# leggedrobotics/elevation_mapping_cupy

Measured on AMD Instinct MI355X. Metric: Mpoints/s fused (map-update p50 latency in config), higher is better.
Workload: dtype f32; 1 GPU; cfg2: 1024x1024 map, 1000000 uniform-random points/frame, core_param.yaml values, add_points + variance fusion, rays/overlap off; index_mode=reference_fp16, cloud=device resident (H2D excluded)

## Files before the change

elevation_mapping_cupy_amd/csrc/emap_api.hip:

```cpp
#include "emap_host.h"
#include <algorithm>
#include <cmath>
#include <cstdio>
#include <cstdlib>
#include <cstring>
#include <new>

using namespace emap_host;

float emap_host::q16(float x) { return (float)(_Float16)x; }
static int frame_impl(emap_ctx* ctx, const float R[9], const float t[3], double position_noise, double orientation_noise, emap_stats* stats, bool sharded);
static void sf_forget_applied(emap_ctx* ctx) {
  const unsigned int passed = ctx->sf_host[0];
  while (ctx->sf_count > 0 && ctx->sf_ring[ctx->sf_head].epoch <= passed) { ctx->sf_head = (ctx->sf_head + 1) % emap_ctx::SF_RING; --ctx->sf_count; }
}
static int sf_recover(emap_ctx* ctx) {
  CK(hipSetDevice(ctx->device));
  CK(hipStreamSynchronize(ctx->stream));
  const unsigned int first = ctx->sf_host[1];
  ctx->sf_host[1] = 0u;
  CK(hipMemset(ctx->sf_poison, 0, 4));
  const BoundCloud bound = ctx->cloud;
  const bool fsem_set = ctx->fsem_set; ctx->fsem_set = false;
  int rc = EMAP_OK;
// ... 242 lines not shown
  hipFree(s->dev);
  *s = Stage{};
}

extern "C" {

int emap_abi_version(void) { return EMAP_ABI_VERSION; }

const char* emap_last_error(const emap_ctx* ctx) { return ctx ? ctx->err.c_str() : "null context"; }

int emap_destroy(emap_ctx* ctx) {
  if (!ctx) return EMAP_OK;
  hipSetDevice(ctx->device);
  if (ctx->post_pending) post_settle(ctx);
  if (ctx->stream) hipStreamSynchronize(ctx->stream);
  hipFree(ctx->cells.hot); hipFree(ctx->cells.cold); hipFree(ctx->acc); hipFree(ctx->accr); hipFree(ctx->trav_in);
  hipFree(ctx->normal); hipFree(ctx->scratch); hipFree(ctx->plug_buf); hipFree(ctx->plug_cnt); hipFree(ctx->slots); hipFree(ctx->frame); hipFree(ctx->cnt_sync);
  for (int k = 0; k < 2; ++k) { hipFree(ctx->pts_dev[k]); if (ctx->pts_pin[k]) hipHostFree(ctx->pts_pin[k]); if (ctx->ev_copied[k]) hipEventDestroy(ctx->ev_copied[k]); if (ctx->ev_used[k]) hipEventDestroy(ctx->ev_used[k]); }
  hipFree(ctx->own_cloud); stage_free(&ctx->cloud_stage); stage_free(&ctx->image_stage);
  if (ctx->copy_stream) hipStreamDestroy(ctx->copy_stream);
  delete ctx->workers;
  hipFree(ctx->tail_idx); hipFree(ctx->tail_flags); hipFree(ctx->ray_S); hipFree(ctx->ray_lut); hipFree(ctx->inert); hipFree(ctx->inl_plane); hipFree(ctx->ray_thr);
  hipFree(ctx->bin_recs); hipFree(ctx->bin_own); hipFree(ctx->bin_own_cnt); hipFree(ctx->bin_hist); hipFree(ctx->bin_tile_total); hipFree(ctx->bin_tile_start); hipFree(ctx->bin_sync); hipFree(ctx->split_mem); hipFree(ctx->sem_split_mem); if (ctx->split_need) hipHostFree((void*)ctx->split_need); if (ctx->sf_host) hipHostFree((void*)ctx->sf_host); hipFree(ctx->frame_save); hipFree(ctx->sf_poison);
  hipFree(ctx->img_uv); hipFree(ctx->img_valid); hipFree(ctx->img_buf);
  hipFree(ctx->grid_buf);
  hipFree(ctx->poly_buf); if (ctx->poly_pin) hipHostFree(ctx->poly_pin);
  hipFree(ctx->sub_tab); hipFree(ctx->sub_out); if (ctx->sub_pin) hipHostFree(ctx->sub_pin);
  hipFree(ctx->cloud_tab); hipFree(ctx->cloud_out); if (ctx->cloud_pin) hipHostFree(ctx->cloud_pin);
  hipFree(ctx->pseg_buf); hipFree(ctx->pseg_slots); if (ctx->pseg_pin) hipHostFree(ctx->pseg_pin);
  hipFree(ctx->terr_buf); if (ctx->terr_pin) hipHostFree(ctx->terr_pin);
  hipFree(ctx->reg_buf); hipFree(ctx->reg_cracks); if (ctx->reg_pin) hipHostFree(ctx->reg_pin);
// ... 397 lines not shown
  if (ctx->pts_bucketed) {
    CKARG(memcmp(ctx->bucket_R, R, sizeof ctx->bucket_R) == 0 && memcmp(ctx->bucket_t, t, sizeof ctx->bucket_t) == 0, "the bound cloud was bucketed for another pose (emap_upload_points_strip)");
    CKARG(ctx->bucket_org_r == ctx->kp.org_r, "the map's rows shifted since the bound cloud was bucketed for this strip (emap_upload_points_strip): upload it again");
  }
  const bool gate_possible = !f || f->gate_possible;
  ctx->bin_rs = 1;
  CK(hipSetDevice(ctx->device));
  const bool binned = ctx->cloud.n > 0 && takes_bins(ctx, ctx->cloud.n_all);
  ctx->frame_binned = binned;
  const bool tm = ctx->stage_timing && f;
  if (binned) {
    int rc = ensure_bins(ctx, ctx->prm.enable_visibility_cleanup != 0, f); if (rc) return rc;
    const Pose pose = make_pose(ctx, R, t);
    BinStg* own = ctx->bin_strip ? reinterpret_cast<BinStg*>(ctx->bin_own) : nullptr;
    if (tm) CK(hipEventRecord(ctx->ev[ST_HIST], ctx->stream));
    bool hist_done = false;
    if (ctx->post_pending) {
      const bool along = f && !tm && !own && ctx->kp.mv.n == 0;
      const bool rays_on = ctx->prm.enable_visibility_cleanup != 0;
      int out = POST_OUT_FULL;
      if (along) {
        out = rays_on ? POST_OUT_TRAV_NORMALS : POST_OUT_TRAV;
        if (const char* e = getenv("EMAP_POST_LEAN")) { if (atoi(e) == 0) out = POST_OUT_FULL; }
      }
      if (along && out == POST_OUT_TRAV && !gate_possible) ctx->post_took = 32;
      else {
        if (along) {
          long max_wg = 0;
          if (const char* e = getenv("EMAP_POST_FUSE_MAX_WG")) max_wg = atol(e);
          hist_done = launch_post_hist(ctx->stream, ctx->device, ctx->kp, ctx->prm.w1, ctx->prm.w2, ctx->prm.w3, ctx->prm.w_out, ctx->cells, ctx->trav_in, ctx->normal,
                                       ctx->ncells_alloc, ctx->prm.dilation_size, pose, ctx->bg, ctx->cloud.pts, ctx->cloud.n, ctx->cloud.stride, ctx->bin_hist, max_wg, out);
        }
        if (hist_done) {
          ++ctx->post_fused;
          if (out == POST_OUT_FULL) ctx->post_pending = false; else ctx->post_took = 16;
          if (out != POST_OUT_TRAV) { ctx->kp.norg_r = ctx->kp.org_r; ctx->kp.norg_c = ctx->kp.org_c; }
          if (out == POST_OUT_FULL) { ctx->torg_r = ctx->kp.org_r; ctx->torg_c = ctx->kp.org_c; }
        } else if ((rc = post_settle(ctx))) return rc;
      }
    }
    if (!hist_done) launch_bin_hist(ctx->stream, ctx->kp, pose, ctx->bg, ctx->cloud.pts, ctx->cloud.n, ctx->cloud.stride, ctx->bin_hist, own, ctx->bin_own_cnt);
    if (tm) CK(hipEventRecord(ctx->ev[ST_SCAN], ctx->stream));
    static const bool split_off = getenv("EMAP_SPLIT") && atoi(getenv("EMAP_SPLIT")) == 0;
    ctx->split.on = gate_possible && !split_off ? 1 : 0;
    {
      static const int cap_forced = getenv("EMAP_SPLIT_CAP") ? atoi(getenv("EMAP_SPLIT_CAP")) : -1;
      static const int pool = getenv("EMAP_SPLIT_POOL") ? atoi(getenv("EMAP_SPLIT_POOL")) : EMAP_SPLIT_POOL_DEFAULT;
      const unsigned int need = *ctx->split_need;
      long cap = need ? (long)need + need / 4 + 8 : 0;
      if (ctx->split.on && cap < pool) cap = pool;
      if (cap_forced >= 0) cap = cap_forced;
      if (cap > (long)SPLIT_MAX_EXTRA) cap = SPLIT_MAX_EXTRA;
      ctx->split.cap = (int)((cap + 7) & ~7L);
    }
    if (ctx->split.on && ctx->split_dirty) {
      CK(hipMemsetAsync(ctx->split_mem, 0, (size_t)SPLIT_MAX_SLOTS * SPLIT_CELLS * 40 + 4 * SPLIT_MAX_SLOTS, ctx->stream));
      ctx->split_dirty = false;
    }
    ctx->split_dirty = ctx->split_dirty || (ctx->split.on != 0 && ctx->split.cap > 0);
    launch_bin_scan(ctx->stream, ctx->bg, ctx->bin_hist, ctx->bin_tile_total, ctx->bin_tile_start, ctx->bin_sync, ctx->split);
    if (tm) CK(hipEventRecord(ctx->ev[ST_SCATTER], ctx->stream));
    launch_bin_scatter(ctx->stream, ctx->kp, pose, ctx->bg, ctx->cloud.pts, ctx->cloud.n, ctx->cloud.stride, ctx->bin_hist, ctx->bin_tile_start, ctx->bin_recs, own, ctx->bin_own_cnt,
                       ctx->cloud.chan, ctx->carry);
    if (tm) CK(hipEventRecord(ctx->ev[ST_GATE], ctx->stream));
    if (gate_possible) launch_tile_count(ctx->stream, ctx->kp, ctx->bg, ctx->bin_recs, ctx->bin_rs, ctx->bin_tile_start, ctx->cells, ctx->slots, ctx->split, ctx->cloud.n);
  } else {
    { const int rc = post_settle(ctx); if (rc) return rc; }
    ctx->carry.on = 0;
    if (tm) for (int e = ST_HIST; e <= ST_SCATTER; ++e) CK(hipEventRecord(ctx->ev[e], ctx->stream));
    static const bool fold_off = getenv("EMAP_GATE_FOLD") && atoi(getenv("EMAP_GATE_FOLD")) == 0;
    const bool fold = f && f->fold_gate && !fold_off && ctx->cnt_sync;
    const bool folded = launch_count(ctx->stream, ctx->kp, make_pose(ctx, R, t), ctx->cloud.pts, ctx->cloud.n, ctx->cloud.stride, ctx->cells, ctx->acc, ctx->slots,
                                     fold ? &f->gate : nullptr, ctx->frame, ctx->cnt_sync);
    if (gate_folded) *gate_folded = folded;
    if (tm) CK(hipEventRecord(ctx->ev[ST_GATE], ctx->stream));
  }
  CK(hipGetLastError());
  return EMAP_OK;
}

// ... 440 lines not shown
```

elevation_mapping_cupy_amd/csrc/emap_binned.hip:

```cpp
#include "emap_launch.h"
#include "emap_bin_hist.h"
#include <cstring>
#include <cstdlib>

#define BIN_QCAP 128


template <int MODE> __device__ __forceinline__ bool row_owned(const KP& P, const Pose& T, float rx, float ry, float rz) {
  const float qx = Qf<MODE>(rx), qy = Qf<MODE>(ry), qz = Qf<MODE>(rz);
  const float x = T.Rq[0] * qx + T.Rq[1] * qy + T.Rq[2] * qz + T.tq[0];
  const int ix = axis_idx<MODE>(P, Qf<MODE>(x));
  return (unsigned int)(phys_row(P, ix) - P.row0) < (unsigned int)P.nrows;
}

struct __attribute__((aligned(16))) BinStg { unsigned int key; float z, v; unsigned int i; };

template <int MODE, int BLK, bool STRIP>
__global__ __launch_bounds__(BLK) void k_bin_hist(KP P, Pose T, BinGeo G, const float* __restrict__ pts, long n, int stride,
                                                  unsigned int* __restrict__ hist, BinStg* __restrict__ stg,
                                                  unsigned int* __restrict__ stg_cnt) {
  extern __shared__ __attribute__((aligned(16))) unsigned int h[];
  if (!STRIP) bin_hist_chunk<MODE, BLK, HIST_U>(P, T, G, pts, n, stride, hist, h, blockIdx.x, gridDim.x);
  else {
    for (int t = threadIdx.x; t < G.TB; t += BLK) h[t] = 0u;
// ... 227 lines not shown
  const unsigned int R0 = tile_start[w.t], R1 = tile_start[w.t + 1], n = R1 - R0;
  w.np = 1u; w.slot = SPLIT_NONE; w.r0 = R0; w.r1 = R1;
  if (SPLIT && n > SPLIT_CAP) {
    const unsigned int sw = SV.tile_slot[w.t];
    if (sw != SPLIT_NONE) {
      w.np = sw >> 16; w.slot = (sw & 0xffffu) + (unsigned int)w.sb;
      const unsigned int len = (n + w.np - 1u) / w.np;
      w.r0 = min(R1, R0 + w.part * len); w.r1 = min(R1, w.r0 + len);
    }
  }
  return true;
}

__device__ __forceinline__ bool drift_inlier(const KP& P, const float4 m, float z) {
  return m.z > 0.5f && (double)fabsf(m.x - z) < (double)m.y * P.mt && (double)m.y < P.dcvi_half && (double)m.w > P.trav_inlier;
}

#define TF_BLOCK 1024
#ifndef SPLIT_U
#define SPLIT_U 4
#endif
#ifndef SPLIT_U_FUSE
#define SPLIT_U_FUSE 1
#endif
__device__ __forceinline__ void stage_hot_tile(const KP& P, Cells cells, float4* s_cell, int row_base, int tx) {
  const int tr = __builtin_amdgcn_readfirstlane(threadIdx.x >> 6), tc = threadIdx.x & 63, lrow = row_base + tr, col = tx * BIN_TC + tc;
  const bool in = lrow < P.nrows && col < P.C;
  const float4* src = cells.hot + ((long)(lrow + P.halo) * P.C + col);
  if (P.mv.n == 0) {
    if (in) lds_dma16(src, s_cell + tr * BIN_TC);
    else s_cell[threadIdx.x] = make_float4(0.f, 0.f, 0.f, 0.f);
  } else {
    float4 m = make_float4(0.f, 0.f, 0.f, 0.f);
    if (in) { m = *src; cell_now(P, m, P.row0 + lrow, col); }
    s_cell[threadIdx.x] = m;
  }
}
template <bool SPLIT, int RS>
__device__ __forceinline__ void tile_count_body(const KP& P, const BinGeo& G, const BinRec* __restrict__ recs, Cells cells,
                                                ErrSlot* __restrict__ slots, const SplitView& SV, const TileWork& w) {
  constexpr int NC = BIN_TR * BIN_TC;
  __shared__ float4 s_cell[NC];
  __shared__ unsigned int s_pts[NC], s_inl[NC];
  const int t = w.t, sb = w.sb;
  const int ty = t / G.tiles_x, tx = t - ty * G.tiles_x;
  const unsigned int r0 = w.r0, r1 = w.r1;
  const int row_base = (ty * G.sub + sb) * BIN_TR;
  if (row_base >= P.nrows || r0 == r1) return;
  const bool split = SPLIT && w.np > 1u;
  constexpr int U = SPLIT ? SPLIT_U : 1;
  BinRec rr[U];
#pragma unroll
  for (int u = 0; u < U; ++u) { const unsigned int k = r0 + u * TF_BLOCK + threadIdx.x; if (k < r1) rr[u] = recs[(size_t)k * RS]; }
  stage_hot_tile(P, cells, s_cell, row_base, tx);
  if (split) { s_pts[threadIdx.x] = 0u; s_inl[threadIdx.x] = 0u; }
  __syncthreads();
  const unsigned int sel = (unsigned int)sb;
  for (unsigned int kb = r0; kb < r1; kb += TF_BLOCK * U) {
    if (kb != r0)
#pragma unroll
    for (int u = 0; u < U; ++u) { const unsigned int k = kb + u * TF_BLOCK + threadIdx.x; if (k < r1) rr[u] = recs[(size_t)k * RS]; }
    long long e_fix = 0; unsigned long long cnt = 0;
#pragma unroll
    for (int u = 0; u < U; ++u) {
      const unsigned int k = kb + u * TF_BLOCK + threadIdx.x;
      bool inl = false;
      if (k < r1) {
        const BinRec& r = rr[u];
        const unsigned int lcb = r.lc_inl & 0x7fffffffu;
        if ((lcb >> 10) == sel) {
          const float4 m = s_cell[lcb & 1023u];
          if (drift_inlier(P, m, r.z)) { inl = true; e_fix += __double2ll_rn((double)(r.z - m.x) * EM_SCALE_E); }
          if (split) { atomicAdd(&s_pts[lcb & 1023u], 1u); if (inl) atomicAdd(&s_inl[lcb & 1023u], 1u); }
        }
      }
      cnt += __popcll(__ballot(inl));
    }
    if (cnt) {
      const long long s = wave_sum_ll(e_fix);
      if ((threadIdx.x & 63) == 0) {
        const unsigned int slot = (unsigned int)(((unsigned int)t * (TF_BLOCK / 64) + (threadIdx.x >> 6) + kb) & (EM_ERR_SLOTS - 1));
        atomicAdd(reinterpret_cast<unsigned long long*>(&slots[slot].sum), (unsigned long long)s);
        atomicAdd(&slots[slot].cnt, cnt);
      }
    }
  }
  if (split) {
    __syncthreads();
    const unsigned int i = w.slot * SPLIT_CELLS + threadIdx.x;
    if (s_pts[threadIdx.x]) atomicAdd(&SV.pts[i], s_pts[threadIdx.x]);
    if (s_inl[threadIdx.x]) atomicAdd(&SV.inl[i], s_inl[threadIdx.x]);
  }
}
template <bool SPLIT, int RS>
__global__ __launch_bounds__(TF_BLOCK) void k_tile_count(KP P, BinGeo G, const BinRec* __restrict__ recs,
                                                          const unsigned int* __restrict__ tile_start, Cells cells,
                                                          ErrSlot* __restrict__ slots, SplitView SV) {
  TileWork w;
  if (tile_work<SPLIT>(G, SV, tile_start, w)) tile_count_body<SPLIT, RS>(P, G, recs, cells, slots, SV, w);
}

template <bool AVG, bool RAYS, bool SPLIT, int RS, bool SEM>
__device__ __forceinline__ void tile_fuse_body(const KP& P, const BinGeo& G, const BinRec* __restrict__ recs, Cells cells,
                                               AccF* __restrict__ acc, FrameDev* __restrict__ F,
                                               unsigned int* __restrict__ cnt_plane, unsigned long long* __restrict__ inert,
                                               unsigned int* __restrict__ inl_plane, float* __restrict__ thr, const OverlapArgs& O, const GateFold& GF,
                                               const SplitView& SV, const TileWork& w, const SemMini& SM) {
  static_assert(!SEM || (AVG && !RAYS && !SPLIT && RS == 2), "the semantic pass rides on whole frames without rays / parts, on 32-byte records");
  constexpr int NC = BIN_TR * BIN_TC;
  struct FuseLds { unsigned int pts[NC], cnt[NC], inl[NC], out[NC]; unsigned long long h[NC], v[NC], latest[NC]; float4 cell[NC]; };
  static_assert(offsetof(FuseLds, cell) == offsetof(FuseLds, h) + 3 * NC * 8 && sizeof(FuseLds) == 56 * NC, "FuseLds is packed");
  __shared__ __attribute__((aligned(16))) FuseLds L;
  unsigned int (&s_pts)[NC] = L.pts; unsigned int (&s_inl)[NC] = L.inl; unsigned int (&s_cnt)[NC] = L.cnt; unsigned int (&s_out)[NC] = L.out;
  unsigned long long (&s_h)[NC] = L.h; unsigned long long (&s_v)[NC] = L.v; unsigned long long (&s_latest)[NC] = L.latest;
// ... 286 lines not shown
  if (own) { if (P.mode == 0) launch_bin_scatter_i<0, BLK, true, false>(s, P, T, G, pts, n, stride, hist, tile_start, recs, own, own_cnt, V, SC); else launch_bin_scatter_i<1, BLK, true, false>(s, P, T, G, pts, n, stride, hist, tile_start, recs, own, own_cnt, V, SC); }
  else if (SC.on) { if (P.mode == 0) launch_bin_scatter_i<0, BLK, false, true>(s, P, T, G, pts, n, stride, hist, tile_start, recs, own, own_cnt, V, SC); else launch_bin_scatter_i<1, BLK, false, true>(s, P, T, G, pts, n, stride, hist, tile_start, recs, own, own_cnt, V, SC); }
  else { if (P.mode == 0) launch_bin_scatter_i<0, BLK, false, false>(s, P, T, G, pts, n, stride, hist, tile_start, recs, own, own_cnt, V, SC); else launch_bin_scatter_i<1, BLK, false, false>(s, P, T, G, pts, n, stride, hist, tile_start, recs, own, own_cnt, V, SC); }
}
void launch_bin_scatter(hipStream_t s, const KP& P, const Pose& T, const BinGeo& G, const float* pts, long n, int stride,
                        const unsigned int* hist, const unsigned int* tile_start, BinRec* recs, const BinStg* own, const unsigned int* own_cnt,
                        const ChanView& V, const SemCarry& SC) {
  static const int blk = env_block("EMAP_SCATTER_BLOCK", 512);
  switch (blk) {
    case 1024: launch_bin_scatter_t<1024>(s, P, T, G, pts, n, stride, hist, tile_start, recs, own, own_cnt, V, SC); break;
    case 512: launch_bin_scatter_t<512>(s, P, T, G, pts, n, stride, hist, tile_start, recs, own, own_cnt, V, SC); break;
    default: launch_bin_scatter_t<256>(s, P, T, G, pts, n, stride, hist, tile_start, recs, own, own_cnt, V, SC);
  }
}
void launch_tile_count(hipStream_t s, const KP& P, const BinGeo& G, const BinRec* recs, int rs, const unsigned int* tile_start, Cells cells,
                       ErrSlot* slots, const SplitView& SV, long n) {
  static_assert(TF_BLOCK == BIN_TR * BIN_TC, "one thread per cell of a tile");
  (void)n;
  const bool split = SV.on && SV.cap > 0;
  const dim3 g((split ? (unsigned int)SV.cap * G.sub : 0u) + tile_grid(G)), b(TF_BLOCK);
  if (split) { if (rs == 2) hipLaunchKernelGGL((k_tile_count<true, 2>), g, b, 0, s, P, G, recs, tile_start, cells, slots, SV); else hipLaunchKernelGGL((k_tile_count<true, 1>), g, b, 0, s, P, G, recs, tile_start, cells, slots, SV); }
  else { if (rs == 2) hipLaunchKernelGGL((k_tile_count<false, 2>), g, b, 0, s, P, G, recs, tile_start, cells, slots, SV); else hipLaunchKernelGGL((k_tile_count<false, 1>), g, b, 0, s, P, G, recs, tile_start, cells, slots, SV); }
}
bool bin_fuse_takes_semantics(const SplitView& SV, bool fuse_average, bool rays, int rs) { return rs == 2 && fuse_average && !rays && !(SV.on && SV.cap > 0); }
#define FUSE_WT_MAX_WGS 1024u
void launch_bin_fuse(hipStream_t s, const KP& P, const BinGeo& G_, const BinRec* recs, int rs, const unsigned int* tile_start, Cells cells,
                     AccF* acc, FrameDev* F, bool fuse_average, bool rays, unsigned int* cnt_plane, unsigned long long* inert,
                     unsigned int* inl_plane, float* thr, const OverlapArgs& O, const GateFold& GF, const SplitView& SV, long n, const SemMini* sm) {
  (void)n;
  const bool split = SV.on && SV.cap > 0;
  BinGeo G = G_;
  const dim3 g((split ? (unsigned int)SV.cap * G.sub : 0u) + tile_grid(G)), b(TF_BLOCK);
  G.wt = g.x <= FUSE_WT_MAX_WGS;
  SemMini SM; memset(&SM, 0, sizeof SM);
#define EM_FUSE_I(A, R, SP, RS_, SE) hipLaunchKernelGGL((k_tile_fuse<A, R, SP, RS_, SE>), g, b, 0, s, P, G, recs, tile_start, cells, acc, F, cnt_plane, inert, inl_plane, thr, O, GF, SV, SM)
// ... 222 lines not shown
```

elevation_mapping_cupy_amd/csrc/emap_host.h:

```cpp
#pragma once
#include "emap_launch.h"
#include "../../include/emap_hip.h"
#include <cmath>
#include <condition_variable>
#include <cstring>
#include <functional>
#include <mutex>
#include <string>
#include <thread>
#include <vector>

enum { ST_HIST = 0, ST_SCAN, ST_SCATTER, ST_GATE, ST_FUSE, ST_COMMIT, ST_RAYS, ST_AVERAGE, ST_OVERLAP, ST_POST, ST_N };

struct RcclApi;
struct ncclComm;

namespace emap_host {
struct Workers {
  std::vector<std::thread> th; std::mutex m; std::condition_variable cv, done_cv;
  std::function<void(int, int)> job; int gen = 0, pending = 0; bool stop = false;
  explicit Workers(int n) {
    for (int i = 0; i < n; ++i) th.emplace_back([this, i, n] {
      int seen = 0;
      for (;;) {
// ... 77 lines not shown
  void* sem_split_mem;
  volatile unsigned int* split_need;
  bool split_dirty;
  unsigned int* cnt_sync;
  unsigned int sf_epoch; volatile unsigned int* sf_host; unsigned int* sf_host_dev; unsigned int* sf_poison;
  FrameDev* frame_save;
  struct SfFrame { unsigned int epoch; float R[9], t[3]; double pn, on; Moves mv; emap_host::BoundCloud cloud; };
  enum { SF_RING = 8 };
  SfFrame sf_ring[SF_RING]; int sf_head, sf_count;
  bool sf_redo;
  unsigned int sf_aborts;
  int update_path;
  bool post_pending;
  int post_took;
  unsigned int post_fused;
  BinGeo bg; BinRec* bin_recs; size_t bin_recs_cap; bool bin_strip;
  float4* bin_own; size_t bin_own_cap; unsigned int* bin_own_cnt;
  unsigned int* bin_hist; size_t bin_hist_cap; unsigned int* bin_tile_total; unsigned int* bin_tile_start;
  bool fsem_set; int fsem_keep_counts; SemSpec fsem;
  int bin_rs; SemCarry carry;
  float* img_uv; unsigned char* img_valid; float* img_buf; size_t img_cap;
  double img_tol; bool img_tol_set;
  float* sem_alpha;
  int sem_layers; float* sem; double* sem_sums; unsigned int* sem_col; unsigned int* cnt_plane;
  float* pts_dev[2]; size_t pts_cap[2];
  float* pts_pin[2]; size_t pin_cap[2];
  hipEvent_t ev_copied[2], ev_used[2];
  int up_slot; bool up_used[2]; hipStream_t copy_stream; emap_host::Workers* workers;
  emap_host::BoundCloud cloud;
  bool pts_bucketed; float bucket_R[9], bucket_t[3]; int bucket_org_r;
// ... 142 lines not shown
```

elevation_mapping_cupy_amd/csrc/emap_kernels.hip:

```cpp
#include "emap_launch.h"
#include "emap_bin_hist.h"
#include <cstdlib>
#include <cstring>

struct CountGate { int on, pad_; GateArgs A; FrameDev* F; unsigned int* sync; };
template <int MODE>
__global__ __launch_bounds__(EM_BLOCK) void k_count(KP P, Pose T, const float* __restrict__ pts, long n, int stride,
                                                     Cells cells, AccF* __restrict__ acc,
                                                     ErrSlot* __restrict__ slots, CountGate CG) {
  long i = (long)blockIdx.x * EM_BLOCK + threadIdx.x;
  long long e_fix = 0;
  unsigned int inl = 0;
  if (i < n) {
    float rx, ry, rz;
    load_point(pts, i, stride, rx, ry, rz);
    Geo g = geometry<MODE>(P, T, rx, ry, rz);
    Owned oc = owned(P, g.ix, g.iy);
    long c = (g.finite && g.valid && g.inside) ? oc.c : -1;
    if (c >= 0) {
      float4 m = cells.hot[c];
      cell_now(P, m, oc.prow, oc.pcol);
      bool inlier = m.z > 0.5f && (double)fabsf(m.x - g.z) < (double)m.y * P.mt && (double)m.y < P.dcvi_half &&
                    (double)m.w > P.trav_inlier;
      if (inlier) { inl = 1; e_fix = __double2ll_rn((double)(g.z - m.x) * EM_SCALE_E); }
// ... 811 lines not shown
        const int dl = q + 1;                                                                                             \
        v2f s01 = {0.f, 0.f}, s23 = {0.f, 0.f};                                                                           \
        _Pragma("unroll") for (int a2 = 0; a2 < 3; ++a2)                                                                  \
          _Pragma("unroll") for (int b2 = 0; b2 < 3; ++b2) {                                                              \
            const float t = (t0)[((a2 - 1) * dl * (dp) + (b2 - 1) * dl) * (ES)];                                          \
            const v2f tt = {t, t};                                                                                        \
            const auto* w = (WT).w[q][a2 * 3 + b2];                                                                       \
            s01 = __builtin_elementwise_fma((v2f){w[0], w[1]}, tt, s01);                                                  \
            s23 = __builtin_elementwise_fma((v2f){w[2], w[3]}, tt, s23);                                                  \
          }                                                                                                               \
        acc = fmaf((WT).wo[q][0], fabsf(s01.x), acc);                                                                       \
        acc = fmaf((WT).wo[q][1], fabsf(s01.y), acc);                                                                       \
        acc = fmaf((WT).wo[q][2], fabsf(s23.x), acc);                                                                       \
        acc = fmaf((WT).wo[q][3], fabsf(s23.y), acc);                                                                       \
      }                                                                                                                   \
      cells.hot[c].w = exp_neg(acc);                                  \
    }                                                                                                                     \
    if (OUT == POST_OUT_TRAV) break;                                                                                      \
    float nx = 0.f, ny = 0.f, nz = 0.f;                                                                                   \
    if ((do_normal) && (own_valid) > 0.5f) {                                           \
      const float dzdx = (t0)[ES] - h, dzdy = (t0)[(ES) * (dp)] - h;                                                      \
      const float ax = -dzdy / P.res_f, ay = -dzdx / P.res_f;            \
      const float nrm = sqrt_rn_ge1((ax * ax) + (ay * ay) + 1.0f);                                                        \
      nx = ax / nrm; ny = ay / nrm; nz = 1.0f / nrm;                                                                      \
    }                                                                                                                     \
    normal[c] = nx; normal[plane_stride + c] = ny; normal[2 * plane_stride + c] = nz;                                     \
  } while (0)

template <int PT_THREADS, class SrcFn>
__device__ __forceinline__ void post_source_masks(unsigned int* __restrict__ sm, int RH, int RW, SrcFn src) {
  constexpr int PT_WAVES = PT_THREADS / 64;
  const int tc = threadIdx.x & 63, wv = __builtin_amdgcn_readfirstlane(threadIdx.x >> 6);
  for (int r = wv; r < RH; r += PT_WAVES) {
// ... 42 lines not shown
  const int s2 = (int)__builtin_ctzll(any) - 2 * d;
  for (int dy = max(-d, s2 - d); dy <= min(d, s2 + d); ++dy) {
    const unsigned int* m = sm + 5 * (R0 + dy) + k;
    if ((__builtin_amdgcn_alignbit(m[1], m[0], sh) >> (s2 - dy + d)) & 1u) { dy_out = dy; dx_out = s2 - dy; return true; }
  }
  return false;
}

struct NullCold { float time, upper, is_upper, valid; };
__device__ const NullCold k_null_cold = {0.f, 0.f, 0.f, 1.f};

template <int PT_R, int STAGE>
__global__ __launch_bounds__(512) void k_post_dma(KP P, TravW Wt, Cells cells, float* __restrict__ trav_in,
                                                  float* __restrict__ normal, long plane_stride, int d, PostSegs S) {
  constexpr int OUT = POST_OUT_FULL;
  int seg_b = S.b[0], seg_e = S.e[0], ty = blockIdx.y;
#pragma unroll
  for (int k = 1; k < 4; ++k) if (k < S.n && (int)blockIdx.y >= S.t0[k]) { seg_b = S.b[k]; seg_e = S.e[k]; ty = blockIdx.y - S.t0[k]; }
  constexpr int PT_THREADS = 512, PT_WAVES = PT_THREADS / 64;
  extern __shared__ __attribute__((aligned(16))) float lds[];
  const int RW = PT_C + 6 + 2 * d, RH = PT_R + 6 + 2 * d, vp = RW + 1;
  const int DW = PT_C + 6, DH = PT_R + 6;
  float4* raw = reinterpret_cast<float4*>(lds);
  float* val = lds + 4 * RH * RW;
  int* rtab = reinterpret_cast<int*>(val + RH * vp);
  unsigned int* hs = reinterpret_cast<unsigned int*>(rtab + ((RH + 3) & ~1));
  unsigned short* holes = reinterpret_cast<unsigned short*>(hs + 8 * RH);
  __shared__ unsigned int n_holes;
  if (threadIdx.x == 0) n_holes = 0u;
  const int C = P.C;
// ... 81 lines not shown
  for (int k = 0; k < RPW; ++k) {
    const int tr = wv * RPW + k, gr = tile_r + tr;
    if (tr >= PT_R || gr >= seg_e) break;
    const int rr = tr + 3 + d, rc = tc + 3 + d;
    const long c = (long)(rtab[rr + 1] & 0xffffff) * C + pcol;
    const float* t0 = &val[rr * vp + rc];
    const float own_valid = raw[rr * RW + rc].w;
    POST_CELL(Wt, 1, t0, vp, own_valid, col_in && gr >= 3 && gr <= C - 4, col_n && gr >= 1 && gr <= C - 3, c);
  }
}

template <int PT_R, int STAGE>
__global__ __launch_bounds__(PT_R >= 32 ? POST_T32 : 512) void k_post(KP P, TravW Wt, Cells cells, float* __restrict__ trav_in,
                                                    float* __restrict__ normal, long plane_stride, int d, PostSegs S) {
  constexpr int OUT = POST_OUT_FULL;
#define POST_BX blockIdx.x
#define POST_BY blockIdx.y
#include "emap_post_tile.h"
#undef POST_BX
#undef POST_BY
}

#ifndef POST_HIST_U
#define POST_HIST_U 4
#endif
template <int MODE, int PT_R, int OUT>
__global__ __launch_bounds__(512) void k_post_hist(KP P, TravW Wt, Cells cells, float* __restrict__ trav_in, float* __restrict__ normal,
                                                   long plane_stride, int d, PostSegs S, int tiles_x, int n_tiles, int tile0, int hist0,
                                                   Pose T, BinGeo G, const float* __restrict__ pts, long n, int stride,
                                                   unsigned int* __restrict__ hist) {
  static_assert(PT_R < 32 || POST_T32 == 512, "k_post_hist runs both bodies with 512 threads");
  const int b = (int)blockIdx.x;
  if ((unsigned int)(b - tile0) < (unsigned int)n_tiles) {
    constexpr int STAGE = 0;
    const unsigned int bx = (unsigned int)((b - tile0) % tiles_x), by = (unsigned int)((b - tile0) / tiles_x);
#define POST_BX bx
#define POST_BY by
#include "emap_post_tile.h"
#undef POST_BX
#undef POST_BY
  } else if ((unsigned int)(b - hist0) < (unsigned int)G.B) {
    extern __shared__ float lds[];
    bin_hist_chunk<MODE, 512, POST_HIST_U>(P, T, G, pts, n, stride, hist, reinterpret_cast<unsigned int*>(lds),
                                           (unsigned int)(b - hist0), (unsigned int)G.B);
  }
// ... 339 lines not shown
  return (R == 16 || R == 32) && !post_launch_dma(P, R, d) && post_lds_bytes(R, d) <= 150 * 1024 ? R : 0;
}
template <auto KERN> static long post_hist_resident(size_t lds, int dev) {
  struct Memo { bool on; size_t lds; long wg; };
  static Memo memo[EM_MAX_DEV];
  Memo& m = memo[dev >= 0 && dev < EM_MAX_DEV ? dev : 0];
  if (m.on && m.lds == lds) return m.wg;
  int per_cu = 0, cus = 0;
  if (hipOccupancyMaxActiveBlocksPerMultiprocessor(&per_cu, reinterpret_cast<const void*>(KERN), 512, lds) != hipSuccess) return 0;
  if (hipDeviceGetAttribute(&cus, hipDeviceAttributeMultiprocessorCount, dev) != hipSuccess) return 0;
  m.on = true; m.lds = lds; m.wg = (long)per_cu * cus;
  return m.wg;
}
bool launch_post_hist(hipStream_t s, int dev, const KP& P, const float* w1, const float* w2, const float* w3, const float* wo, Cells cells,
                      float* trav_in, float* normal, long plane_stride, int d, const Pose& T, const BinGeo& G, const float* pts, long n, int stride,
                      unsigned int* hist, long max_wg, int out) {
  const int R = post_hist_tile_rows(P, d);
  if (!R) return false;
  const TravW W = post_weights(w1, w2, w3, wo);
  PostSegs S; memset(&S, 0, sizeof S);
  S.emagic = post_emagic(d);
  S.n = 1; S.b[0] = 0; S.e[0] = P.C; S.t0[0] = 0;
  static const bool hist_front = getenv("EMAP_POST_HIST_FRONT") && atoi(getenv("EMAP_POST_HIST_FRONT")) != 0;
  const int tiles_x = (P.C + PT_C - 1) / PT_C, n_tiles = tiles_x * ((P.C + R - 1) / R);
  const int tile0 = hist_front ? (G.B + 7) & ~7 : 0, hist0 = hist_front ? 0 : (n_tiles + 7) & ~7;
  const long grid = hist_front ? (long)tile0 + n_tiles : (long)hist0 + G.B;
  const size_t hist_lds = sizeof(unsigned int) * (size_t)G.pitch, lds = post_lds_bytes(R, d) > hist_lds ? post_lds_bytes(R, d) : hist_lds;
  if (lds > 158 * 1024) return false;
  bool ok = false;
#define POST_HIST_GO(MODE, RR, OO) do { auto kern = k_post_hist<MODE, RR, OO>; static LdsRaised raised; \
    if (!raise_lds(kern, raised, 158 * 1024) && lds > 64 * 1024) break; \
    const long room = post_hist_resident<k_post_hist<MODE, RR, OO>>(lds, dev); \
    if (grid > (max_wg > 0 && max_wg < room ? max_wg : room)) break; \
    hipLaunchKernelGGL(kern, dim3((unsigned int)grid), dim3(512), lds, s, P, W, cells, trav_in, normal, plane_stride, d, S, tiles_x, n_tiles, tile0, hist0, \
                       T, G, pts, n, stride, hist); ok = true; } while (0)
#define POST_HIST_OUT(MODE, RR) do { if (out == POST_OUT_TRAV) POST_HIST_GO(MODE, RR, POST_OUT_TRAV); \
    else if (out == POST_OUT_TRAV_NORMALS) POST_HIST_GO(MODE, RR, POST_OUT_TRAV_NORMALS); else POST_HIST_GO(MODE, RR, POST_OUT_FULL); } while (0)
  if (P.mode == 0) { if (R == 32) POST_HIST_OUT(0, 32); else POST_HIST_OUT(0, 16); }
  else { if (R == 32) POST_HIST_OUT(1, 32); else POST_HIST_OUT(1, 16); }
#undef POST_HIST_OUT
#undef POST_HIST_GO
  return ok;
}
void launch_var_time(hipStream_t s, const KP& P, Cells cells, int do_var, int do_time) {
  hipLaunchKernelGGL(k_var_time, dim3(nblk((long)P.nrows * P.C)), dim3(EM_BLOCK), 0, s, P, cells, do_var, do_time);
}
void launch_publish(hipStream_t s, const KP& P, Cells cells, const float* normal, long plane_stride, int kind, float center_z,
                    int only_above, float* out) {
  const long M = P.C - 2;
  hipLaunchKernelGGL(k_publish, dim3(nblk(M * M)), dim3(EM_BLOCK), 0, s, P, cells, normal, plane_stride, kind, center_z, only_above, out);
}
// ... 24 lines not shown
```

elevation_mapping_cupy_amd/csrc/emap_launch.h:

```cpp
#pragma once
#include "emap_device.h"
#include <cstddef>

struct SemRaw { int op, stride, K, n_max; long size, cells; double alpha; };
struct CamArgs { float P[12], K[9], D[5], center[3]; float x1, y1, z1, ih, iw; double tol; };
#define EM_CAM_CELL_MAX 65536
struct CmaxSpec { int n; int chan[8]; int layer[8]; };
struct DepthArgs { int H, W, step, Hs, Ws, has_rgb, n_feat; long n, plane; float fx, fy, cx, cy, depth_scale, min_depth, max_depth, conf_thr;
                   const void* depth; const float* conf; const unsigned char* rgb; const float* feat; float* xyz; float* chan; };
#define EM_DEPTH_MAX_SIDE 8192
#define EM_DEPTH_MAX_STEP 64
#define EM_DEPTH_MAX_CHAN 16
#define EM_CLOUDMSG_MAX_COLS 19
#define EM_CLOUDMSG_MAX_STEP 256
#define EM_CLOUDMSG_MAX_POINTS (1L << 26)
#define EM_CLOUDMSG_STAGE_BYTES 16384
struct CloudMsgArgs { const unsigned char* msg; float* xyz; float* chan; long row_step; int rows, width, point_step, n_cols, tile, tiles_per_row;
                      unsigned int col[EM_CLOUDMSG_MAX_COLS]; };
static inline int cloud_unpack_tile(int point_step) {
  int t = 1024;
  while (t > 64 && (long)t * point_step > EM_CLOUDMSG_STAGE_BYTES) t >>= 1;
  return t;
}
#define EM_IMGMSG_MAX_SIDE 8192
// ... 18 lines not shown
                        const GateArgs&, FrameDev*, FrameDev*, ErrSlot*, unsigned int*, unsigned int*, unsigned int*, unsigned int*, unsigned int, unsigned int, int);
void launch_fuse(hipStream_t, const KP&, const Pose&, const float*, long, int, Cells, AccF*, const FrameDev*);
void launch_commit(hipStream_t, const KP&, Cells, const AccF*, const FrameDev*, unsigned long long*);
void launch_rays(hipStream_t, const KP&, const Pose&, const RayTab&, const float*, long, int, Cells, const AccRView&, const float*, long, FrameDev*, bool, const unsigned long long*, const unsigned int*, int, const float*, const unsigned int*, const unsigned int*);
void launch_win_pack(hipStream_t, const KP&, const Win&, Cells, const float*, long, const unsigned int*, const unsigned long long*, float);
void launch_win_prepare(hipStream_t, const Win&, int);
void launch_win_unpack(hipStream_t, const KP&, const Win&, AccR*);
void launch_win_reduce(hipStream_t, long long*, unsigned int*, const long long*, const unsigned int*, int, long, long, long);
void launch_ray_apply(hipStream_t, const KP&, Cells, AccR*, unsigned long long*, const OverlapArgs&, FrameDev*, unsigned int*, int);
void launch_average(hipStream_t, const KP&, Cells, AccF*, AccR*, const FrameDev*, bool, bool, unsigned int*, const OverlapArgs&);
void launch_overlap(hipStream_t, const KP&, Cells, int, int, float, float);
void launch_var_time(hipStream_t, const KP&, Cells, int, int);
int post_tile_rows(const KP&);
void launch_post(hipStream_t, const KP&, const float*, const float*, const float*, const float*, Cells, float*, float*, long, int, int, const int*, const int*, int, int);
int post_hist_tile_rows(const KP&, int);
enum { POST_OUT_FULL = 0, POST_OUT_TRAV_NORMALS = 1, POST_OUT_TRAV = 2 };
bool launch_post_hist(hipStream_t, int, const KP&, const float*, const float*, const float*, const float*, Cells, float*, float*, long, int,
                      const Pose&, const BinGeo&, const float*, long, int, unsigned int*, long, int);
void launch_get_plane(hipStream_t, const KP&, Cells, int, float*);
void launch_publish(hipStream_t, const KP&, Cells, const float*, long, int, float, int, float*);
void launch_set_plane(hipStream_t, const KP&, Cells, int, const float*);
void launch_fill_cells(hipStream_t, Cells, long, const Cell&);
void launch_point_index(hipStream_t, const KP&, const Pose&, const float*, long, int, int*, unsigned char*);
void launch_plane_view(hipStream_t, const KP&, int, int, float*, float*, int);
void launch_materialize(hipStream_t, const KP&, Cells);
void launch_band_clear(hipStream_t, const KP&, float*, int, long, int, int);

void launch_sem_points(hipStream_t, const KP&, const Pose&, const SemSpec&, const float*, long, int, const ChanView&, double*, unsigned int*, long);
void launch_sem_finalize(hipStream_t, const KP&, const SemSpec&, const unsigned int*, double*, unsigned int*, float*, float*, long);
void launch_semraw_acc(hipStream_t, const SemRaw&, const float*, const int*, const int*, const float*, const int*, float*, unsigned int*);
void launch_semraw_fin(hipStream_t, const SemRaw&, float*, const unsigned int*, const int*, const float*, const float*, float*);
void launch_polygon_mask(hipStream_t, int, const int*, const int*, int, const int*, float*);
void launch_dilate_planes(hipStream_t, int, int, const float*, const float*, float*, float*);
void launch_cmax_ids(hipStream_t, const KP&, const CmaxSpec&, const ChanView&, long, const float*, long, unsigned char*, unsigned char*);
void launch_cmax_sum(hipStream_t, const KP&, const Pose&, const CmaxSpec&, const float*, long, int, const ChanView&, const int*, long long*, long);
void launch_cmax_select(hipStream_t, const KP&, const CmaxSpec&, int, const long long*, long, unsigned char*, unsigned char*, const unsigned int*, float*, float*, float*);
void launch_image_corr(hipStream_t, const KP&, const CamArgs&, Cells, float*, unsigned char*);
void launch_image_fuse(hipStream_t, const KP&, int, float*, const float*, const float*, const unsigned char*, float, float, double);
void launch_inpaint_sweep(hipStream_t, int, const float*, const float*, float*, float*, const unsigned int*, unsigned int*);
void launch_min_sweep(hipStream_t, int, int, const float*, const float*, const float*, float*, float*, const unsigned int*, unsigned int*, bool);
void launch_box3(hipStream_t, int, const float*, float*);
void launch_erode(hipStream_t, int, int, const float*, float*);

void launch_bin_hist(hipStream_t, const KP&, const Pose&, const BinGeo&, const float*, long, int, unsigned int*, BinStg*, unsigned int*);
void launch_bin_scan(hipStream_t, const BinGeo&, unsigned int*, unsigned int*, unsigned int*, unsigned int*, const SplitView&);
void launch_bin_scatter(hipStream_t, const KP&, const Pose&, const BinGeo&, const float*, long, int, const unsigned int*, const unsigned int*, BinRec*, const BinStg*, const unsigned int*, const ChanView&, const SemCarry&);
void launch_tile_count(hipStream_t, const KP&, const BinGeo&, const BinRec*, int, const unsigned int*, Cells, ErrSlot*, const SplitView&, long);
void launch_tile_semantic(hipStream_t, const KP&, const BinGeo&, const SemSpec&, const BinRec*, int, int, const unsigned int*, const ChanView&, long,
                          const unsigned int*, float*, float*, long, const SplitView&, void*, int);
size_t sem_split_bytes(int);
bool sem_split_possible(const SemSpec&);
void launch_bin_fuse(hipStream_t, const KP&, const BinGeo&, const BinRec*, int, const unsigned int*, Cells, AccF*, FrameDev*, bool, bool, unsigned int*, unsigned long long*, unsigned int*, float*, const OverlapArgs&, const GateFold&, const SplitView&, long, const SemMini*);
bool bin_fuse_takes_semantics(const SplitView&, bool, bool, int);

void launch_depth_cloud(hipStream_t, const DepthArgs&, int);

void launch_cloud_unpack(hipStream_t, const CloudMsgArgs&, bool aligned4);

static inline int image_frame_variant(int esize) { return esize == 1 ? 0 : esize == 2 ? 1 : esize == 4 ? 2 : 3; }
void launch_image_frame(hipStream_t, const KP&, const CamArgs&, Cells, float*, unsigned char*, const ImgMsgArgs&, float*, long);

void launch_grid_map(hipStream_t, const KP&, Cells, const GridArgs&);
// ... 109 lines not shown
```

Baseline: 17790 Mpoints/s.

## Write traversability inlier flags as bytes in fused post pass for tile count

In the trav-only fused post+histogram pass, instead of writing the full float traversability into the hot cell word, the kernel writes a one-byte above/below/unchanged flag per cell into a new buffer. The tile-count kernel then reads these flags to decide drift inliers instead of relying on the updated traversability word. This is meant to cut the post pass's write traffic to the 16-byte hot cells and so lower memory traffic on the critical path. It adds a byte-plane allocation, a new kernel variant and an environment switch, and traversability stays deferred in the hot cells.

```diff
diff --git a/elevation_mapping_cupy_amd/csrc/emap_api.hip b/elevation_mapping_cupy_amd/csrc/emap_api.hip
--- a/elevation_mapping_cupy_amd/csrc/emap_api.hip
+++ b/elevation_mapping_cupy_amd/csrc/emap_api.hip
@@ -280,7 +280,7 @@
   hipSetDevice(ctx->device);
   if (ctx->post_pending) post_settle(ctx);
   if (ctx->stream) hipStreamSynchronize(ctx->stream);
-  hipFree(ctx->cells.hot); hipFree(ctx->cells.cold); hipFree(ctx->acc); hipFree(ctx->accr); hipFree(ctx->trav_in);
+  hipFree(ctx->cells.hot); hipFree(ctx->cells.cold); hipFree(ctx->acc); hipFree(ctx->accr); hipFree(ctx->trav_in); hipFree(ctx->trav_flag);
   hipFree(ctx->normal); hipFree(ctx->scratch); hipFree(ctx->plug_buf); hipFree(ctx->plug_cnt); hipFree(ctx->slots); hipFree(ctx->frame); hipFree(ctx->cnt_sync);
   for (int k = 0; k < 2; ++k) { hipFree(ctx->pts_dev[k]); if (ctx->pts_pin[k]) hipHostFree(ctx->pts_pin[k]); if (ctx->ev_copied[k]) hipEventDestroy(ctx->ev_copied[k]); if (ctx->ev_used[k]) hipEventDestroy(ctx->ev_used[k]); }
   hipFree(ctx->own_cloud); stage_free(&ctx->cloud_stage); stage_free(&ctx->image_stage);
@@ -708,7 +708,7 @@
     const Pose pose = make_pose(ctx, R, t);
     BinStg* own = ctx->bin_strip ? reinterpret_cast<BinStg*>(ctx->bin_own) : nullptr;
     if (tm) CK(hipEventRecord(ctx->ev[ST_HIST], ctx->stream));
-    bool hist_done = false;
+    bool hist_done = false, flags_written = false;
     if (ctx->post_pending) {
       const bool along = f && !tm && !own && ctx->kp.mv.n == 0;
       const bool rays_on = ctx->prm.enable_visibility_cleanup != 0;
@@ -717,18 +717,29 @@
         out = rays_on ? POST_OUT_TRAV_NORMALS : POST_OUT_TRAV;
         if (const char* e = getenv("EMAP_POST_LEAN")) { if (atoi(e) == 0) out = POST_OUT_FULL; }
       }
-      if (along && out == POST_OUT_TRAV && !gate_possible) ctx->post_took = 32;
+      const bool trav_only = out == POST_OUT_TRAV;
+      if (along && trav_only && !gate_possible) ctx->post_took = 32;
       else {
+        if (trav_only) {
+          if (const char* e = getenv("EMAP_POST_FLAGS")) { if (atoi(e) == 0) out = POST_OUT_TRAV_WORD; }
+          if (out == POST_OUT_TRAV && !ctx->trav_flag) {
+            unsigned char* pl = nullptr;
+            CK(hipMalloc((void**)&pl, (size_t)ctx->ncells_alloc));
+            if (hipMemsetAsync(pl, TRAV_FLAG_WORD, (size_t)ctx->ncells_alloc, ctx->stream) != hipSuccess) { hipFree(pl); ctx->err = "hipMemsetAsync(trav_flag)"; return EMAP_ERR_HIP; }
+            ctx->trav_flag = pl;
+          }
+        }
         if (along) {
           long max_wg = 0;
           if (const char* e = getenv("EMAP_POST_FUSE_MAX_WG")) max_wg = atol(e);
           hist_done = launch_post_hist(ctx->stream, ctx->device, ctx->kp, ctx->prm.w1, ctx->prm.w2, ctx->prm.w3, ctx->prm.w_out, ctx->cells, ctx->trav_in, ctx->normal,
-                                       ctx->ncells_alloc, ctx->prm.dilation_size, pose, ctx->bg, ctx->cloud.pts, ctx->cloud.n, ctx->cloud.stride, ctx->bin_hist, max_wg, out);
+                                       ctx->ncells_alloc, ctx->prm.dilation_size, pose, ctx->bg, ctx->cloud.pts, ctx->cloud.n, ctx->cloud.stride, ctx->bin_hist, max_wg, out, ctx->trav_flag);
         }
         if (hist_done) {
           ++ctx->post_fused;
+          flags_written = out == POST_OUT_TRAV;
           if (out == POST_OUT_FULL) ctx->post_pending = false; else ctx->post_took = 16;
-          if (out != POST_OUT_TRAV) { ctx->kp.norg_r = ctx->kp.org_r; ctx->kp.norg_c = ctx->kp.org_c; }
+          if (!trav_only) { ctx->kp.norg_r = ctx->kp.org_r; ctx->kp.norg_c = ctx->kp.org_c; }
           if (out == POST_OUT_FULL) { ctx->torg_r = ctx->kp.org_r; ctx->torg_c = ctx->kp.org_c; }
         } else if ((rc = post_settle(ctx))) return rc;
       }
@@ -757,7 +768,8 @@
     launch_bin_scatter(ctx->stream, ctx->kp, pose, ctx->bg, ctx->cloud.pts, ctx->cloud.n, ctx->cloud.stride, ctx->bin_hist, ctx->bin_tile_start, ctx->bin_recs, own, ctx->bin_own_cnt,
                        ctx->cloud.chan, ctx->carry);
     if (tm) CK(hipEventRecord(ctx->ev[ST_GATE], ctx->stream));
-    if (gate_possible) launch_tile_count(ctx->stream, ctx->kp, ctx->bg, ctx->bin_recs, ctx->bin_rs, ctx->bin_tile_start, ctx->cells, ctx->slots, ctx->split, ctx->cloud.n);
+    if (gate_possible) launch_tile_count(ctx->stream, ctx->kp, ctx->bg, ctx->bin_recs, ctx->bin_rs, ctx->bin_tile_start, ctx->cells, ctx->slots, ctx->split, ctx->cloud.n,
+                                         flags_written ? ctx->trav_flag : nullptr);
   } else {
     { const int rc = post_settle(ctx); if (rc) return rc; }
     ctx->carry.on = 0;
diff --git a/elevation_mapping_cupy_amd/csrc/emap_binned.hip b/elevation_mapping_cupy_amd/csrc/emap_binned.hip
--- a/elevation_mapping_cupy_amd/csrc/emap_binned.hip
+++ b/elevation_mapping_cupy_amd/csrc/emap_binned.hip
@@ -265,6 +265,10 @@
 
 __device__ __forceinline__ bool drift_inlier(const KP& P, const float4 m, float z) {
   return m.z > 0.5f && (double)fabsf(m.x - z) < (double)m.y * P.mt && (double)m.y < P.dcvi_half && (double)m.w > P.trav_inlier;
+}
+__device__ __forceinline__ bool drift_inlier(const KP& P, const float4 m, float z, unsigned int flag) {
+  const bool trav = flag == TRAV_FLAG_WORD ? (double)m.w > P.trav_inlier : flag != TRAV_FLAG_BELOW;
+  return m.z > 0.5f && (double)fabsf(m.x - z) < (double)m.y * P.mt && (double)m.y < P.dcvi_half && trav;
 }
 
 #define TF_BLOCK 1024
@@ -287,11 +291,13 @@
     s_cell[threadIdx.x] = m;
   }
 }
-template <bool SPLIT, int RS>
+template <bool SPLIT, int RS, bool FLAGS>
 __device__ __forceinline__ void tile_count_body(const KP& P, const BinGeo& G, const BinRec* __restrict__ recs, Cells cells,
-                                                ErrSlot* __restrict__ slots, const SplitView& SV, const TileWork& w) {
+                                                ErrSlot* __restrict__ slots, const SplitView& SV, const TileWork& w,
+                                                const unsigned char* __restrict__ tflag) {
   constexpr int NC = BIN_TR * BIN_TC;
   __shared__ float4 s_cell[NC];
+  __shared__ unsigned char s_flag[FLAGS ? NC : 1];
   __shared__ unsigned int s_pts[NC], s_inl[NC];
   const int t = w.t, sb = w.sb;
   const int ty = t / G.tiles_x, tx = t - ty * G.tiles_x;
@@ -303,7 +309,13 @@
   BinRec rr[U];
 #pragma unroll
   for (int u = 0; u < U; ++u) { const unsigned int k = r0 + u * TF_BLOCK + threadIdx.x; if (k < r1) rr[u] = recs[(size_t)k * RS]; }
+  unsigned char fl = TRAV_FLAG_WORD;
+  if (FLAGS) {
+    const int lrow = row_base + (int)(threadIdx.x >> 6), col = tx * BIN_TC + (int)(threadIdx.x & 63);
+    if (lrow < P.nrows && col < P.C) fl = tflag[(long)(lrow + P.halo) * P.C + col];
+  }
   stage_hot_tile(P, cells, s_cell, row_base, tx);
+  if (FLAGS) s_flag[threadIdx.x] = fl;
   if (split) { s_pts[threadIdx.x] = 0u; s_inl[threadIdx.x] = 0u; }
   __syncthreads();
   const unsigned int sel = (unsigned int)sb;
@@ -321,7 +333,7 @@
         const unsigned int lcb = r.lc_inl & 0x7fffffffu;
         if ((lcb >> 10) == sel) {
           const float4 m = s_cell[lcb & 1023u];
-          if (drift_inlier(P, m, r.z)) { inl = true; e_fix += __double2ll_rn((double)(r.z - m.x) * EM_SCALE_E); }
+          if (FLAGS ? drift_inlier(P, m, r.z, (unsigned int)s_flag[lcb & 1023u]) : drift_inlier(P, m, r.z)) { inl = true; e_fix += __double2ll_rn((double)(r.z - m.x) * EM_SCALE_E); }
           if (split) { atomicAdd(&s_pts[lcb & 1023u], 1u); if (inl) atomicAdd(&s_inl[lcb & 1023u], 1u); }
         }
       }
@@ -348,7 +360,14 @@
                                                           const unsigned int* __restrict__ tile_start, Cells cells,
                                                           ErrSlot* __restrict__ slots, SplitView SV) {
   TileWork w;
-  if (tile_work<SPLIT>(G, SV, tile_start, w)) tile_count_body<SPLIT, RS>(P, G, recs, cells, slots, SV, w);
+  if (tile_work<SPLIT>(G, SV, tile_start, w)) tile_count_body<SPLIT, RS, false>(P, G, recs, cells, slots, SV, w, nullptr);
+}
+template <bool SPLIT, int RS>
+__global__ __launch_bounds__(TF_BLOCK) void k_tile_count_flags(KP P, BinGeo G, const BinRec* __restrict__ recs,
+                                                                const unsigned int* __restrict__ tile_start, Cells cells,
+                                                                ErrSlot* __restrict__ slots, SplitView SV, const unsigned char* __restrict__ tflag) {
+  TileWork w;
+  if (tile_work<SPLIT>(G, SV, tile_start, w)) tile_count_body<SPLIT, RS, true>(P, G, recs, cells, slots, SV, w, tflag);
 }
 
 template <bool AVG, bool RAYS, bool SPLIT, int RS, bool SEM>
@@ -665,11 +684,16 @@
   }
 }
 void launch_tile_count(hipStream_t s, const KP& P, const BinGeo& G, const BinRec* recs, int rs, const unsigned int* tile_start, Cells cells,
-                       ErrSlot* slots, const SplitView& SV, long n) {
+                       ErrSlot* slots, const SplitView& SV, long n, const unsigned char* trav_flag) {
   static_assert(TF_BLOCK == BIN_TR * BIN_TC, "one thread per cell of a tile");
   (void)n;
   const bool split = SV.on && SV.cap > 0;
   const dim3 g((split ? (unsigned int)SV.cap * G.sub : 0u) + tile_grid(G)), b(TF_BLOCK);
+  if (trav_flag) {
+    if (split) { if (rs == 2) hipLaunchKernelGGL((k_tile_count_flags<true, 2>), g, b, 0, s, P, G, recs, tile_start, cells, slots, SV, trav_flag); else hipLaunchKernelGGL((k_tile_count_flags<true, 1>), g, b, 0, s, P, G, recs, tile_start, cells, slots, SV, trav_flag); }
+    else { if (rs == 2) hipLaunchKernelGGL((k_tile_count_flags<false, 2>), g, b, 0, s, P, G, recs, tile_start, cells, slots, SV, trav_flag); else hipLaunchKernelGGL((k_tile_count_flags<false, 1>), g, b, 0, s, P, G, recs, tile_start, cells, slots, SV, trav_flag); }
+    return;
+  }
   if (split) { if (rs == 2) hipLaunchKernelGGL((k_tile_count<true, 2>), g, b, 0, s, P, G, recs, tile_start, cells, slots, SV); else hipLaunchKernelGGL((k_tile_count<true, 1>), g, b, 0, s, P, G, recs, tile_start, cells, slots, SV); }
   else { if (rs == 2) hipLaunchKernelGGL((k_tile_count<false, 2>), g, b, 0, s, P, G, recs, tile_start, cells, slots, SV); else hipLaunchKernelGGL((k_tile_count<false, 1>), g, b, 0, s, P, G, recs, tile_start, cells, slots, SV); }
 }
diff --git a/elevation_mapping_cupy_amd/csrc/emap_host.h b/elevation_mapping_cupy_amd/csrc/emap_host.h
--- a/elevation_mapping_cupy_amd/csrc/emap_host.h
+++ b/elevation_mapping_cupy_amd/csrc/emap_host.h
@@ -115,6 +115,7 @@
   bool post_pending;
   int post_took;
   unsigned int post_fused;
+  unsigned char* trav_flag;
   BinGeo bg; BinRec* bin_recs; size_t bin_recs_cap; bool bin_strip;
   float4* bin_own; size_t bin_own_cap; unsigned int* bin_own_cnt;
   unsigned int* bin_hist; size_t bin_hist_cap; unsigned int* bin_tile_total; unsigned int* bin_tile_start;
diff --git a/elevation_mapping_cupy_amd/csrc/emap_kernels.hip b/elevation_mapping_cupy_amd/csrc/emap_kernels.hip
--- a/elevation_mapping_cupy_amd/csrc/emap_kernels.hip
+++ b/elevation_mapping_cupy_amd/csrc/emap_kernels.hip
@@ -849,9 +849,11 @@
         acc = fmaf((WT).wo[q][2], fabsf(s23.x), acc);                                                                       \
         acc = fmaf((WT).wo[q][3], fabsf(s23.y), acc);                                                                       \
       }                                                                                                                   \
-      cells.hot[c].w = exp_neg(acc);                                  \
-    }                                                                                                                     \
-    if (OUT == POST_OUT_TRAV) break;                                                                                      \
+      const float tv = exp_neg(acc);                                                                                      \
+      if (OUT == POST_OUT_TRAV) tflag[c] = (double)tv > P.trav_inlier ? TRAV_FLAG_ABOVE : TRAV_FLAG_BELOW;    \
+      else cells.hot[c].w = tv;                                       \
+    } else if (OUT == POST_OUT_TRAV) tflag[c] = TRAV_FLAG_WORD;                 \
+    if (OUT == POST_OUT_TRAV || OUT == POST_OUT_TRAV_WORD) break;                                                         \
     float nx = 0.f, ny = 0.f, nz = 0.f;                                                                                   \
     if ((do_normal) && (own_valid) > 0.5f) {                                           \
       const float dzdx = (t0)[ES] - h, dzdy = (t0)[(ES) * (dp)] - h;                                                      \
@@ -924,6 +926,7 @@
 __global__ __launch_bounds__(512) void k_post_dma(KP P, TravW Wt, Cells cells, float* __restrict__ trav_in,
                                                   float* __restrict__ normal, long plane_stride, int d, PostSegs S) {
   constexpr int OUT = POST_OUT_FULL;
+  constexpr unsigned char* tflag = nullptr;
   int seg_b = S.b[0], seg_e = S.e[0], ty = blockIdx.y;
 #pragma unroll
   for (int k = 1; k < 4; ++k) if (k < S.n && (int)blockIdx.y >= S.t0[k]) { seg_b = S.b[k]; seg_e = S.e[k]; ty = blockIdx.y - S.t0[k]; }
@@ -1035,6 +1038,7 @@
 __global__ __launch_bounds__(PT_R >= 32 ? POST_T32 : 512) void k_post(KP P, TravW Wt, Cells cells, float* __restrict__ trav_in,
                                                     float* __restrict__ normal, long plane_stride, int d, PostSegs S) {
   constexpr int OUT = POST_OUT_FULL;
+  constexpr unsigned char* tflag = nullptr;
 #define POST_BX blockIdx.x
 #define POST_BY blockIdx.y
 #include "emap_post_tile.h"
@@ -1049,7 +1053,7 @@
 __global__ __launch_bounds__(512) void k_post_hist(KP P, TravW Wt, Cells cells, float* __restrict__ trav_in, float* __restrict__ normal,
                                                    long plane_stride, int d, PostSegs S, int tiles_x, int n_tiles, int tile0, int hist0,
                                                    Pose T, BinGeo G, const float* __restrict__ pts, long n, int stride,
-                                                   unsigned int* __restrict__ hist) {
+                                                   unsigned int* __restrict__ hist, unsigned char* __restrict__ tflag) {
   static_assert(PT_R < 32 || POST_T32 == 512, "k_post_hist runs both bodies with 512 threads");
   const int b = (int)blockIdx.x;
   if ((unsigned int)(b - tile0) < (unsigned int)n_tiles) {
@@ -1419,9 +1423,9 @@
 }
 bool launch_post_hist(hipStream_t s, int dev, const KP& P, const float* w1, const float* w2, const float* w3, const float* wo, Cells cells,
                       float* trav_in, float* normal, long plane_stride, int d, const Pose& T, const BinGeo& G, const float* pts, long n, int stride,
-                      unsigned int* hist, long max_wg, int out) {
+                      unsigned int* hist, long max_wg, int out, unsigned char* tflag) {
   const int R = post_hist_tile_rows(P, d);
-  if (!R) return false;
+  if (!R || (out == POST_OUT_TRAV && !tflag)) return false;
   const TravW W = post_weights(w1, w2, w3, wo);
   PostSegs S; memset(&S, 0, sizeof S);
   S.emagic = post_emagic(d);
@@ -1438,8 +1442,9 @@
     const long room = post_hist_resident<k_post_hist<MODE, RR, OO>>(lds, dev); \
     if (grid > (max_wg > 0 && max_wg < room ? max_wg : room)) break; \
     hipLaunchKernelGGL(kern, dim3((unsigned int)grid), dim3(512), lds, s, P, W, cells, trav_in, normal, plane_stride, d, S, tiles_x, n_tiles, tile0, hist0, \
-                       T, G, pts, n, stride, hist); ok = true; } while (0)
+                       T, G, pts, n, stride, hist, tflag); ok = true; } while (0)
 #define POST_HIST_OUT(MODE, RR) do { if (out == POST_OUT_TRAV) POST_HIST_GO(MODE, RR, POST_OUT_TRAV); \
+    else if (out == POST_OUT_TRAV_WORD) POST_HIST_GO(MODE, RR, POST_OUT_TRAV_WORD); \
     else if (out == POST_OUT_TRAV_NORMALS) POST_HIST_GO(MODE, RR, POST_OUT_TRAV_NORMALS); else POST_HIST_GO(MODE, RR, POST_OUT_FULL); } while (0)
   if (P.mode == 0) { if (R == 32) POST_HIST_OUT(0, 32); else POST_HIST_OUT(0, 16); }
   else { if (R == 32) POST_HIST_OUT(1, 32); else POST_HIST_OUT(1, 16); }
diff --git a/elevation_mapping_cupy_amd/csrc/emap_launch.h b/elevation_mapping_cupy_amd/csrc/emap_launch.h
--- a/elevation_mapping_cupy_amd/csrc/emap_launch.h
+++ b/elevation_mapping_cupy_amd/csrc/emap_launch.h
@@ -56,9 +56,10 @@
 int post_tile_rows(const KP&);
 void launch_post(hipStream_t, const KP&, const float*, const float*, const float*, const float*, Cells, float*, float*, long, int, int, const int*, const int*, int, int);
 int post_hist_tile_rows(const KP&, int);
-enum { POST_OUT_FULL = 0, POST_OUT_TRAV_NORMALS = 1, POST_OUT_TRAV = 2 };
+enum { POST_OUT_FULL = 0, POST_OUT_TRAV_NORMALS = 1, POST_OUT_TRAV = 2, POST_OUT_TRAV_WORD = 3 };
+enum { TRAV_FLAG_BELOW = 0, TRAV_FLAG_ABOVE = 1, TRAV_FLAG_WORD = 2 };
 bool launch_post_hist(hipStream_t, int, const KP&, const float*, const float*, const float*, const float*, Cells, float*, float*, long, int,
-                      const Pose&, const BinGeo&, const float*, long, int, unsigned int*, long, int);
+                      const Pose&, const BinGeo&, const float*, long, int, unsigned int*, long, int, unsigned char*);
 void launch_get_plane(hipStream_t, const KP&, Cells, int, float*);
 void launch_publish(hipStream_t, const KP&, Cells, const float*, long, int, float, int, float*);
 void launch_set_plane(hipStream_t, const KP&, Cells, int, const float*);
@@ -87,7 +88,8 @@
 void launch_bin_hist(hipStream_t, const KP&, const Pose&, const BinGeo&, const float*, long, int, unsigned int*, BinStg*, unsigned int*);
 void launch_bin_scan(hipStream_t, const BinGeo&, unsigned int*, unsigned int*, unsigned int*, unsigned int*, const SplitView&);
 void launch_bin_scatter(hipStream_t, const KP&, const Pose&, const BinGeo&, const float*, long, int, const unsigned int*, const unsigned int*, BinRec*, const BinStg*, const unsigned int*, const ChanView&, const SemCarry&);
-void launch_tile_count(hipStream_t, const KP&, const BinGeo&, const BinRec*, int, const unsigned int*, Cells, ErrSlot*, const SplitView&, long);
+void launch_tile_count(hipStream_t, const KP&, const BinGeo&, const BinRec*, int, const unsigned int*, Cells, ErrSlot*, const SplitView&, long,
+                       const unsigned char* trav_flag);
 void launch_tile_semantic(hipStream_t, const KP&, const BinGeo&, const SemSpec&, const BinRec*, int, int, const unsigned int*, const ChanView&, long,
                           const unsigned int*, float*, float*, long, const SplitView&, void*, int);
 size_t sem_split_bytes(int);
```

Result: faster. 18220 Mpoints/s (median of 6 runs) (+2.5%).
